# wenet-e2e/wenet

Measured on AMD Instinct MI355X. Metric: audio-seconds/sec (RTF^-1), 12L Conformer fbank80, ctc_prefix_beam_search, higher is better.
Workload: dtype f32 (feed-forward and subsampling-conv2 GEMMs: fp32 operands as three exact bf16 planes, six plane products on the bf16 matrix cores, f32 accumulate -- error <= the v_mfma_f32 kernel's, tests/test_gpu_x6.py; everything else v_mfma_f32)

## Files before the change

wenet_amd/csrc/cabi_ops.hip:

```cpp
#include "model_state.h"
#include "x6.h"

namespace wn {
namespace {

__global__ __launch_bounds__(256) void conv1_image_unpack_kernel(
    const char* __restrict__ img, int tiles, const int* __restrict__ t1_off,
    const int* __restrict__ t1_len, int F1, int C, float* __restrict__ out) {
  const int b = blockIdx.y;
  const int n = t1_len[b] * F1 * (C / 8);
  const int ne = (F1 + 1) / 2;
  for (int i = blockIdx.x * 256 + threadIdx.x; i < n; i += gridDim.x * 256) {
    const int cg = i % (C / 8), px = i / (C / 8);
    const int fr = px / F1, pos = px - fr * F1;
    const int f1 = pos < ne ? 2 * pos : 2 * (pos - ne) + 1;
    const int row = (t1_off[b] + fr) * F1;
    const char* src = img + x3_piece(cg >> 1, tiles, row + pos, cg & 1);
    const bf16x8 p0 = *reinterpret_cast<const bf16x8*>(src);
    const bf16x8 p1 = *reinterpret_cast<const bf16x8*>(src + X3_REC);
    const bf16x8 p2 = *reinterpret_cast<const bf16x8*>(src + 2 * X3_REC);
    float* o = out + ((int64_t)row + f1) * C + cg * 8;
#pragma unroll
    for (int e = 0; e < 8; ++e) o[e] = ((float)p0[e] + (float)p1[e]) + (float)p2[e];
  }
// ... 176 lines not shown
  a.B3 = w3.as<char>(); a.M = M; a.N = N; a.K = K; a.bm = bm;
  if (bm == 120) { a.bm = 128; a.nw = 8; }
  if (bm == 129) { a.bm = 128; a.nw = 4; }
  a.bias = bias; a.resid = resid; a.ldr = N; a.alpha = alpha; a.act = act; a.C = C; a.ldc = N;
  for (int r = 0; r < (reps > 0 ? reps : 1); ++r) WN_TRY(gemm_x6(a, s));
  return 0;
}

int wn_op_ffn_x6(const float* X, const float* W1, const float* b1, const float* W2,
                 const float* b2, float* x, const float* ln_w, const float* ln_b, float* y,
                 int32_t M, int32_t D, int32_t F, int32_t act, float alpha, float eps,
                 int32_t reps, void* stream) {
  WN_CHECK(X && W1 && b1 && W2 && b2 && x && ln_w && ln_b && y, "ffn_x6: null argument");
  WN_CHECK(M > 0 && (D == 256 || D == 512) && F > 0 && F % 64 == 0, "ffn_x6: shape");
  hipStream_t s = (hipStream_t)stream;
  static thread_local DevBuf x3, w13, w23, h3, part;
  if (tune().ffn_x6f != 0 && tune().x6_af32 == 0 && ffn_x6f_supported(M, D, F, act)) {
    FfnX6Args a;
    a.S = ffn_x6f_split(M, F);
    WN_TRY(w13.ensure(x6_bytes(F, D)));
    WN_TRY(w23.ensure(x6_bytes(D, F)));
    WN_TRY(part.ensure((size_t)a.S * M * D * sizeof(float)));
    WN_TRY(x6_split(W1, F, D, D, w13.as<char>(), s));
    WN_TRY(x6_split_perm(W2, D, F, F, w23.as<char>(), s));
    a.X = X; a.ldx = D; a.W13 = w13.as<char>(); a.W2p = w23.as<char>(); a.b1 = b1;
    a.P = part.as<float>(); a.M = M; a.D = D; a.F = F; a.act = act;
    if (tune().ffn_ximg == 2) {
      WN_TRY(x3.ensure(x6_bytes(M, D)));
      WN_TRY(x6_split(X, M, D, D, x3.as<char>(), s));
      a.X3 = x3.as<char>(); a.X = nullptr;
    }
    for (int r = 0; r < (reps > 0 ? reps : 1); ++r) WN_TRY(ffn_x6f(a, s));
    return ffn_reduce_ln(x, part.as<float>(), a.S, b2, alpha, ln_w, ln_b, nullptr, nullptr, y, M,
                         D, eps, 0, s);
  }
  const int S = ffn_x6_split(M, F);
  WN_TRY(x3.ensure(x6_bytes(M, D)));
  WN_TRY(w13.ensure(x6_bytes(F, D)));
  WN_TRY(w23.ensure(x6_bytes(D, F)));
  WN_TRY(h3.ensure(x6_bytes(M, F)));
  WN_TRY(part.ensure((size_t)S * M * D * sizeof(float)));
  WN_TRY(x6_split(W1, F, D, D, w13.as<char>(), s));
  WN_TRY(x6_split(W2, D, F, F, w23.as<char>(), s));
  const bool af32 = tune().x6_af32 != 0 && (int64_t)M * F * 4 < ((int64_t)1 << 31);
  static thread_local DevBuf hf;
  if (af32) WN_TRY(hf.ensure((size_t)M * F * sizeof(float)));
  for (int r = 0; r < (reps > 0 ? reps : 1); ++r) {
// ... 844 lines not shown
```

wenet_amd/csrc/conformer.hip:

```cpp
#include <algorithm>
#include "model_state.h"

namespace {
struct ProfBracket {
  wn_model* m;
  hipStream_t s;
  bool on = false;
  int record(int which) { WN_HIP(hipEventRecord(m->prof_ev[m->prof_used + which], s)); return 0; }
  int begin() {
    on = m->prof_on && (m->prof_seq++ % m->prof_stride) == 0;
    if (!on) return 0;
    if (m->prof_used + 2 > m->prof_ev.size())
      for (int i = 0; i < 64; ++i) {
        hipEvent_t e;
        WN_HIP(hipEventCreate(&e));
        m->prof_ev.push_back(e);
      }
    return record(0);
  }
  int end(double flops, const char* kernel) {
    if (!on) return 0;
    WN_TRY(record(1));
    m->prof_used += 2;
    m->prof_flops += flops;
// ... 87 lines not shown
static void* t1_image_for(wn_model* m, const Linear& w1, const Linear& w2, int act) {
  if (tune().ffn_ximg == 0) return nullptr;
  const int r = ffn_x6_route(m, w1, w2, act);
  if (r == 0 || (r == 2 && tune().x6_af32 != 0)) return nullptr;
  if (m->t1_img.ensure(x6_bytes(m->rows, m->cfg.d_model)) != 0) return nullptr;
  return m->t1_img.p;
}

static int ffn_x6_try(wn_model* m, const Linear& w1, const Linear& w2, int act, hipStream_t s) {
  const ModelData& W = *m->data;
  const int d = m->cfg.d_model, M = m->rows, F = w1.out;
  const bool ximg = m->t1_img_ok;
  m->t1_img_ok = false;
  const int route = ffn_x6_route(m, w1, w2, act);
  WN_CHECK(route != 0 || !ximg,
           "ffn_x6_try: LN(x) was left as a plane image but no six-product form takes it");
  if (route == 0) return 0;
  auto i1 = W.x6_at.find(w1.w), i2 = W.x6_at.find(w2.w);
  ProfBracket pb{m, s};
  if (route == 1) {
    FfnX6Args a;
    a.S = ffn_x6f_split(M, F);
    if (m->ffn_part.ensure((size_t)a.S * M * d * sizeof(float)) != 0) return -1;
    a.X = m->t1.as<float>(); a.ldx = d; a.W13 = i1->second; a.W2p = W.x6p_at.find(w2.w)->second;
    a.b1 = w1.b;
    if (ximg) { a.X3 = m->t1_img.p; a.X = nullptr; }
    a.P = m->ffn_part.as<float>(); a.M = M; a.D = d; a.F = F; a.act = act;
    WN_TRY(pb.begin());
    if (ffn_x6f(a, s) != 0) return -1;
    WN_TRY(pb.end(4.0 * M * (double)F * d,
                  "ffn_x6f_kernel (FFN w_1 + act + w_2, six bf16 plane products)"));
    m->prof_split = a.S;
    return a.S;
  }
  const int S = ffn_x6_split(M, F);
  if (m->ffn_part.ensure((size_t)S * M * d * sizeof(float)) != 0) return -1;
  const bool af32 = tune().x6_af32 != 0 && (int64_t)M * F * 4 < ((int64_t)1 << 31);
  X6Args g1;
  g1.B3 = i1->second; g1.M = M; g1.N = F; g1.K = d; g1.bias = w1.b; g1.act = act;
  if (af32) {
    WN_CHECK(!ximg, "ffn_x6_try: LN(x) was left as a plane image, x6_af32 wants fp32 rows");
    if (m->hbuf.ensure((size_t)M * F * sizeof(float)) != 0) return -1;
    g1.A = m->t1.as<float>(); g1.lda = d; g1.a_bytes = (int64_t)M * d * 4;
    g1.epi = 0; g1.C = m->hbuf.as<float>(); g1.ldc = F;
  } else {
    if (m->x6_h.ensure(x6_bytes(M, F)) != 0 || (!ximg && m->x6_a.ensure(x6_bytes(M, d)) != 0)) return -1;
    if (!ximg && x6_split(m->t1.as<float>(), M, d, d, m->x6_a.as<char>(), s) != 0) return -1;
// ... 424 lines not shown
```

wenet_amd/csrc/ffn_x6f.hip:

```cpp
#include <type_traits>

#include "common.h"
#include "gemm_epilogue.h"
#include "kernels.h"
#include "x6.h"

namespace wn {

namespace {

__device__ unsigned long long g_x6f_clk[4][24];

constexpr int REC = X3_REC;
constexpr int XSTAGE = 24 * REC;
constexpr int XD = 256;
constexpr int XKB = XD / 16;

typedef unsigned u32x4 __attribute__((ext_vector_type(4)));
struct Frag6 { bf16x8 p[2][3]; };

__global__ __launch_bounds__(256) void x6_split_perm_kernel(const float* __restrict__ src, int R,
                                                            int K, int ld,
                                                            char* __restrict__ dst) {
  const int tiles = (R + 31) >> 5, nkb = K >> 4;
  const int64_t idx = (int64_t)blockIdx.x * 256 + threadIdx.x;
  const int row_l = (int)(idx & 31), h = (int)((idx >> 5) & 1);
  const int64_t rest = idx >> 6;
  const int kb = (int)(rest % nkb), tile = (int)(rest / nkb);
  if (tile >= tiles) return;
  const int row = tile * 32 + row_l;
  f32x4 a = {0.f, 0.f, 0.f, 0.f}, b = a;
  if (row < R) {
    const float* s = src + (int64_t)row * ld + kb * 16 + h * 4;
    a = *reinterpret_cast<const f32x4*>(s);
    b = *reinterpret_cast<const f32x4*>(s + 8);
  }
  bf16x8 p0, p1, p2;
#pragma unroll
  for (int e = 0; e < 4; ++e) {
    const Split3 sa = split3(a[e]), sb = split3(b[e]);
    p0[e] = sa.h0; p1[e] = sa.h1; p2[e] = sa.h2;
    p0[4 + e] = sb.h0; p1[4 + e] = sb.h1; p2[4 + e] = sb.h2;
  }
  char* o = dst + ((int64_t)kb * tiles + tile) * X3_TILE + h * 512 + row_l * 16;
  *reinterpret_cast<bf16x8*>(o) = p0;
  *reinterpret_cast<bf16x8*>(o + REC) = p1;
  *reinterpret_cast<bf16x8*>(o + 2 * REC) = p2;
}

__device__ __forceinline__ void wait_vm_stages(int stages) {
  switch (stages) {
    case 0: asm volatile("s_waitcnt vmcnt(0)" ::: "memory"); break;
    case 1: asm volatile("s_waitcnt vmcnt(6)" ::: "memory"); break;
    case 2: asm volatile("s_waitcnt vmcnt(12)" ::: "memory"); break;
    case 3: asm volatile("s_waitcnt vmcnt(18)" ::: "memory"); break;
    default: asm volatile("s_waitcnt vmcnt(24)" ::: "memory"); break;
  }
}

template <int ACT, int RING, int VAR>
__global__ __launch_bounds__(256, 1) void ffn_x6f_kernel(FfnX6Args p, int tiles_m, int pairmap) {
  extern __shared__ __attribute__((aligned(16))) char smem_g[];
  typedef __attribute__((address_space(3))) void* lds_ptr;
  constexpr int HALF = (VAR & 512) ? 2 : 1;
  constexpr int STG = XSTAGE * HALF;
  constexpr int SPC = 8 / HALF;
  static_assert(RING >= 3 && RING * STG <= 6 * XSTAGE, "ring of at most 144 KB");
  float* b1s = reinterpret_cast<float*>(smem_g + RING * STG);

  const int bid = blockIdx.x, xcd = bid & 7, rr = bid >> 3;
  int slice, tm;
  if (pairmap && p.S >= 2 && p.S <= 8) {
    const int nsp = p.S >> 1, pair = xcd % nsp, tg = xcd / nsp;
    slice = 2 * pair + (rr & 1);
    tm = (rr >> 1) * (8 / nsp) + tg;
  } else if (p.S <= 8) {
    slice = xcd & (p.S - 1);
    tm = rr * (8 / p.S) + xcd / p.S;
  } else {
    const int sub = p.S >> 3;
    slice = xcd + 8 * (rr % sub);
    tm = rr / sub;
  }
  if (tm >= tiles_m) return;

  unsigned long long clk[20] = {0, 0, 0, 0, 0, 0, 0, 0, 0, 0, 0, 0, 0, 0, 0, 0, 0, 0, 0, 0};
  if constexpr ((VAR & 8192) != 0) {
    clk[9] = __builtin_readcyclecounter();
    clk[12] = __builtin_amdgcn_s_memrealtime();
  }
  const int tid = threadIdx.x, lane = tid & 63;
  const int wave = __builtin_amdgcn_readfirstlane(tid >> 6);
  __builtin_assume(wave >= 0 && wave < 4);
  const int hi = lane >> 5, li = lane & 31;
  const int NC = p.F / p.S / 64;
  const int cg0 = slice * NC;
  const int FT = p.F >> 5;
  const unsigned vlane = (unsigned)lane * 16u;

  const __amdgpu_buffer_rsrc_t r1 = __builtin_amdgcn_make_buffer_rsrc(
      const_cast<char*>(reinterpret_cast<const char*>(p.W13)), 0,
      (int)((int64_t)p.F * XD * 6), 0x00020000);
  const __amdgpu_buffer_rsrc_t r2 = __builtin_amdgcn_make_buffer_rsrc(
      const_cast<char*>(reinterpret_cast<const char*>(p.W2p)), 0,
      (int)((int64_t)p.F * XD * 6), 0x00020000);

  auto issue_sub = [&](int c, int sub, int buf) {
    char* dst = smem_g + buf * STG + (sub % HALF) * XSTAGE + wave * 6 * REC;
    const int cg = cg0 + c;
    if (sub < 4) {
      const int nt = sub >> 1;
#pragma unroll
      for (int j2 = 0; j2 < 2; ++j2) {
        const int ks = (sub & 1) * 8 + wave * 2 + j2;
        const int so = ((ks * FT + 2 * cg + nt) * 3) * REC;
#pragma unroll
        for (int pl = 0; pl < 3; ++pl)
// ... 25 lines not shown
      __builtin_amdgcn_raw_ptr_buffer_load_lds(r2, (lds_ptr)dst, 16, vlane, so + j * REC, 0, 0);
    }
  };
  auto read_group = [&](int buf, int g) {
    const char* st = smem_g + buf * STG + g * 6 * REC + lane * 16;
    Frag6 f;
#pragma unroll
    for (int t = 0; t < 2; ++t)
#pragma unroll
      for (int pl = 0; pl < 3; ++pl)
        f.p[t][pl] = *reinterpret_cast<const bf16x8*>(st + (t * 3 + pl) * REC);
    return f;
  };

  constexpr bool XT = (VAR & 16384) != 0;
  constexpr bool XI = (VAR & 32768) != 0;
  bf16x8 X[XKB][3];
  const int xrow = min(tm * 128 + wave * 32 + li, p.M - 1);
  f32x4 xa[XKB], xb[XKB];
  f32x4 xr[4][8];
  if constexpr (XI) {
    const int tiles = (p.M + 31) >> 5;
    const int tile = min(tm * 4 + wave, tiles - 1);
    const char* xi = reinterpret_cast<const char*>(p.X3) + (int64_t)tile * X3_TILE + lane * 16;
    const int64_t kstr = (int64_t)tiles * X3_TILE;
#pragma unroll
    for (int ks = 0; ks < XKB; ++ks)
#pragma unroll
      for (int pl = 0; pl < 3; ++pl)
        X[ks][pl] = *reinterpret_cast<const bf16x8*>(xi + ks * kstr + pl * REC);
  } else if constexpr (XT) {
    const int r4 = lane >> 4, c16 = lane & 15;
#pragma unroll
    for (int q = 0; q < 4; ++q)
#pragma unroll
      for (int j = 0; j < 8; ++j) {
        const int row = min(tm * 128 + wave * 32 + 4 * j + r4, p.M - 1);
        xr[q][j] = *reinterpret_cast<const f32x4*>(p.X + (int64_t)row * p.ldx + q * 64 + c16 * 4);
      }
  } else {
    const float* xr0 = p.X + (int64_t)xrow * p.ldx + hi * 8;
#pragma unroll
    for (int ks = 0; ks < XKB; ++ks) {
      xa[ks] = *reinterpret_cast<const f32x4*>(xr0 + ks * 16);
      xb[ks] = *reinterpret_cast<const f32x4*>(xr0 + ks * 16 + 4);
    }
  }
#pragma unroll
  for (int t = 0; t < ((VAR & 16384) ? RING - 1 : RING); ++t) issue(0, t, t);
  float b1v[8];
#pragma unroll
  for (int i = 0; i < 8; ++i) b1v[i] = p.b1[cg0 * 64 + min(tid + 256 * i, NC * 64 - 1)];
  if constexpr ((VAR & 8192) != 0) { __builtin_amdgcn_sched_barrier(0); clk[15] = __builtin_readcyclecounter(); __builtin_amdgcn_sched_barrier(0); }
  if constexpr (XT && !XI) {
    char* patch = smem_g + (RING - 1) * STG + wave * (32 * 272);
    const int r4 = lane >> 4, c16 = lane & 15;
#pragma unroll
    for (int q = 0; q < 4; ++q) {
#pragma unroll
      for (int j = 0; j < 8; ++j)
        *reinterpret_cast<f32x4*>(patch + (4 * j + r4) * 272 + c16 * 16) = xr[q][j];
#pragma unroll
      for (int k4 = 0; k4 < 4; ++k4) {
        xa[4 * q + k4] = *reinterpret_cast<const f32x4*>(patch + li * 272 + k4 * 64 + hi * 32);
        xb[4 * q + k4] = *reinterpret_cast<const f32x4*>(patch + li * 272 + k4 * 64 + hi * 32 + 16);
      }
      asm volatile("s_waitcnt lgkmcnt(0)" ::: "memory");
    }
  }
  if constexpr (!XI) {
#pragma unroll
    for (int ks = 0; ks < XKB; ++ks) {
#pragma unroll
      for (int e = 0; e < 4; ++e) {
        const Split3 sa = split3(xa[ks][e]), sb = split3(xb[ks][e]);
        X[ks][0][e] = sa.h0; X[ks][1][e] = sa.h1; X[ks][2][e] = sa.h2;
        X[ks][0][4 + e] = sb.h0; X[ks][1][4 + e] = sb.h1; X[ks][2][4 + e] = sb.h2;
      }
    }
  }
  if constexpr ((VAR & 8192) != 0) { __builtin_amdgcn_sched_barrier(0); clk[16] = __builtin_readcyclecounter(); __builtin_amdgcn_sched_barrier(0); }
  asm volatile("s_waitcnt vmcnt(0)" ::: "memory");
  if constexpr ((VAR & 8192) != 0) { __builtin_amdgcn_sched_barrier(0); clk[17] = __builtin_readcyclecounter(); __builtin_amdgcn_sched_barrier(0); }
#pragma unroll
  for (int ks = 0; ks < XKB; ++ks)
#pragma unroll
    for (int pl = 0; pl < 3; ++pl) asm volatile("" : "+v"(X[ks][pl]));
#pragma unroll
  for (int i = 0; i < 8; ++i)
    if (tid + 256 * i < NC * 64) b1s[tid + 256 * i] = b1v[i];
  __syncthreads();
  if constexpr ((VAR & 8192) != 0) { __builtin_amdgcn_sched_barrier(0); clk[18] = __builtin_readcyclecounter(); __builtin_amdgcn_sched_barrier(0); }

  f32x16 Y[8];
#pragma unroll
  for (int i = 0; i < 8; ++i)
#pragma unroll
    for (int r = 0; r < 16; ++r) Y[i][r] = 0.f;
  f32x16 HE[2], HO[2];
  u32x4 Hp[4][3];
  if (VAR & 4)
#pragma unroll
    for (int i = 0; i < 12; ++i) {
      Hp[i / 3][i % 3] = u32x4{0x3f803f80u, 0x3f803f80u, 0x3f803f80u, 0x3f803f80u};
      asm volatile("" : "+v"(Hp[i / 3][i % 3]));
    }

  constexpr int PW[6] = {2, 0, 1, 1, 0, 0}, PX[6] = {0, 2, 1, 0, 1, 0};
  constexpr int RT[6] = {0, 1, 0, 1, 0, 1}, RP[6] = {2, 2, 0, 0, 1, 1};

  float pv0 = 0.f, pv1 = 0.f, pt0 = 0.f, pt1 = 0.f;
  unsigned ph0 = 0, ph1 = 0;
  auto pk = [](float a, float b) {
    typedef __bf16 bf16x2 __attribute__((ext_vector_type(2)));
    const bf16x2 h = {(__bf16)a, (__bf16)b};
    return __builtin_bit_cast(unsigned, h);
  };
  auto lo = [](unsigned u) { return __builtin_bit_cast(float, u << 16); };
  auto hi16 = [](unsigned u) { return __builtin_bit_cast(float, u & 0xffff0000u); };
  auto piece_slice = [&](int nt, int i, int k, const f32x4& bq) {
    const int r = 2 * i;
    switch (k) {
      case 0: {
        float b0 = bq[r & 3];
        asm volatile("" : "+v"(b0));
        pv0 = HE[nt][r] + b0;
        break;
      }
      case 1: {
        float b1 = bq[(r + 1) & 3];
        asm volatile("" : "+v"(b1), "+v"(pv0));
        pv0 += HO[nt][r];
        pv1 = HE[nt][r + 1] + b1;
        break;
      }
      case 2:
        asm volatile("" : "+v"(pv0), "+v"(pv1));
        pv1 += HO[nt][r + 1];
        if (ACT == ACT_SILU) pt0 = pv0 * -1.4426950408889634f;
        break;
      case 3:
        if (ACT == ACT_SILU) {
          asm volatile("" : "+v"(pt0), "+v"(pv1));
          pt1 = pv1 * -1.4426950408889634f;
          pt0 = wn_exp2(pt0);
        }
        break;
      case 4:
        if (ACT == ACT_SILU) {
          asm volatile("" : "+v"(pt0), "+v"(pt1));
          pt1 = wn_exp2(pt1);
          pt0 = 1.0f + pt0;
        }
        break;
      case 5:
        if (ACT == ACT_SILU) {
          asm volatile("" : "+v"(pt0), "+v"(pt1));
          pt1 = 1.0f + pt1;
          pt0 = wn_rcp(pt0);
        }
        break;
// ... 9 lines not shown
      case 7:
        asm volatile("" : "+v"(pv0), "+v"(pv1));
        if (ACT == ACT_SILU) {
          asm volatile("" : "+v"(pt1));
          pv1 *= pt1;
        }
        if (ACT == ACT_RELU) pv1 = fmaxf(pv1, 0.0f);
        ph0 = pk(pv0, pv1);
        break;
      case 8:
        asm volatile("" : "+v"(pv0), "+v"(pv1), "+v"(ph0));
        pv0 -= lo(ph0); pv1 -= hi16(ph0);
        break;
      case 9:
        asm volatile("" : "+v"(pv0), "+v"(pv1));
        ph1 = pk(pv0, pv1);
        break;
      case 10:
        asm volatile("" : "+v"(pv0), "+v"(pv1), "+v"(ph1));
        pv0 -= lo(ph1); pv1 -= hi16(ph1);
        break;
      default: {
        asm volatile("" : "+v"(pv0), "+v"(pv1));
        const int kb = 2 * nt + (r >> 3), d = (r & 7) >> 1;
        Hp[kb][0][d] = ph0;
        Hp[kb][1][d] = ph1;
        Hp[kb][2][d] = pk(pv0, pv1);
        break;
      }
    }
  };
  auto read_frag = [&](int b, int g, int t, int pl) {
    return *reinterpret_cast<const bf16x8*>(smem_g + b * STG + (g * 6 + t * 3 + pl) * REC +
                                            lane * 16);
  };
  const f32x16 zero16 = {0.f, 0.f, 0.f, 0.f, 0.f, 0.f, 0.f, 0.f, 0.f, 0.f, 0.f, 0.f, 0.f, 0.f, 0.f,
                         0.f};

  int buf = 0;
  Frag6 fc;
#pragma unroll
  for (int q = 0; q < 6; ++q) fc.p[RT[q]][RP[q]] = read_frag(0, 0, RT[q], RP[q]);
  if constexpr ((VAR & 8192) != 0) clk[10] = __builtin_readcyclecounter();
  auto chunk = [&](auto last_tag, int c) {
    constexpr bool last = decltype(last_tag)::value;
    f32x4 bq = {0.f, 0.f, 0.f, 0.f};
#pragma unroll
    for (int sub = 0; sub < 8; ++sub) {
      if constexpr ((VAR & 8192) != 0 && !last) {
        __builtin_amdgcn_sched_barrier(0);
        clk[sub] = __builtin_readcyclecounter();
        __builtin_amdgcn_sched_barrier(0);
      }
#pragma unroll
      for (int g = 0; g < 4; ++g) {
        Frag6 fn;
        const bool do_piece = sub >= 2 && sub < 6;
        const int pnt = sub >= 4 ? 1 : 0;
        const int pi = ((sub & 1) << 2) + g;
        if (do_piece && (pi & 1) == 0)
          bq = *reinterpret_cast<const f32x4*>(b1s + c * 64 + pnt * 32 + 8 * (pi >> 1) + 4 * hi);
#pragma unroll
        for (int k = 0; k < 12; ++k) {
          const int q = k >> 1, tl = k & 1;
          if ((VAR & 1) || ((VAR & 65536) && q >= 3)) {
            asm volatile("" ::"v"(fc.p[tl][PW[q]]));
          } else if (sub < 4) {
            const int nt = sub >> 1, ks = (sub & 1) * 8 + 2 * g + tl;
            const bool first = (sub & 1) == 0 && g == 0 && q == 0;
            f32x16& H = tl == 0 ? HE[nt] : HO[nt];
            H = __builtin_amdgcn_mfma_f32_32x32x16_bf16(fc.p[tl][PW[q]], X[ks][PX[q]],
                                                       first ? zero16 : H, 0, 0, 0);
          } else {
            const bf16x8 hb = __builtin_bit_cast(bf16x8, Hp[sub - 4][PX[q]]);
            Y[2 * g + tl] = __builtin_amdgcn_mfma_f32_32x32x16_bf16(fc.p[tl][PW[q]], hb,
                                                                    Y[2 * g + tl], 0, 0, 0);
          }
          const int st = sub / HALF;
          const bool sync_sub = sub % HALF == HALF - 1;
          const int gs = (sub % HALF) * 4 + g;
          if (g == 3 && k == 5 && sync_sub) {
            __builtin_amdgcn_sched_barrier(0);
            if (!(VAR & 8)) {
              if (!(VAR & 1024)) {
                asm volatile("s_waitcnt lgkmcnt(0)" ::: "memory");
                const int tail = SPC - 2 - st < 0 ? 0 : (SPC - 2 - st > RING - 2 ? RING - 2 : SPC - 2 - st);
                if (last) wait_vm_stages(tail * HALF); else wait_vm_stages((RING - 2) * HALF);
              }
              if (!(VAR & 2048)) __builtin_amdgcn_s_barrier();
// ... 2 lines not shown
              if (st + RING < SPC) issue(c, st + RING, buf);
              else if (!last) issue(c + 1, st + RING - SPC, buf);
            }
            buf = buf + 1 == RING ? 0 : buf + 1;
            __builtin_amdgcn_sched_barrier(0);
          }
          if constexpr ((VAR & 16384) != 0 && !(VAR & 2)) {
            static_assert(!(VAR & 16384) || HALF == 2, "spread DMA: 48-record stages");
            const int ka = do_piece ? 9 : 2, kb = do_piece ? 11 : 8;
            if ((k == ka || k == kb) && gs < 6) {
              const int j12 = gs * 2 + (k == kb ? 1 : 0);
              const int tst = st + RING - 1;
              const int bufp = buf == 0 ? RING - 1 : buf - 1;
              if (tst < SPC) issue_one(c, tst * HALF + j12 / 6, bufp, j12 % 6);
              else if (!last) issue_one(c + 1, (tst - SPC) * HALF + j12 / 6, bufp, j12 % 6);
            }
          }
          if (VAR & 64) {
            fn = fc;
          } else if (g < 3 || !sync_sub) {
            if (VAR & 4096) {
              if (k == 0)
#pragma unroll
                for (int i = 0; i < 6; ++i) fn.p[RT[i]][RP[i]] = read_frag(buf, gs + 1, RT[i], RP[i]);
            } else if (tl == 1) {
              fn.p[RT[q]][RP[q]] = read_frag(buf, gs + 1, RT[q], RP[q]);
            }
          } else if (k >= 6 && (sub < 7 || !last)) {
            fn.p[RT[k - 6]][RP[k - 6]] = read_frag(buf, 0, RT[k - 6], RP[k - 6]);
          }
          if (do_piece) {
            if (VAR & 4) {
              if (k == 11) {
                const int r = 2 * pi, kb = 2 * pnt + (r >> 3), d = (r & 7) >> 1;
                Hp[kb][0][d] = __builtin_bit_cast(unsigned, HE[pnt][r]) & 0x3f803f80u;
                Hp[kb][1][d] = __builtin_bit_cast(unsigned, HO[pnt][r]) & 0x3f803f80u;
                Hp[kb][2][d] = __builtin_bit_cast(unsigned, HE[pnt][r + 1]) & 0x3f803f80u;
              }
            } else {
              piece_slice(pnt, pi, k, bq);
            }
          }
          __builtin_amdgcn_sched_barrier(0);
        }
        fc = fn;
      }
    }
    if constexpr ((VAR & 8192) != 0 && !last) clk[8] = __builtin_readcyclecounter();
  };
  for (int c = 0; c + 1 < NC; ++c) chunk(std::false_type{}, c);
  chunk(std::true_type{}, NC - 1);

  if constexpr ((VAR & 8192) != 0) clk[11] = __builtin_readcyclecounter();
  const int row = tm * 128 + wave * 32 + li;
  if constexpr (XT) {
    __syncthreads();
    char* patch = smem_g + wave * (32 * 1040);
#pragma unroll
    for (int i = 0; i < 8; ++i)
#pragma unroll
      for (int g = 0; g < 4; ++g)
        *reinterpret_cast<f32x4*>(patch + li * 1040 + (i * 32 + 8 * g + 4 * hi) * 4) =
            f32x4{Y[i][4 * g], Y[i][4 * g + 1], Y[i][4 * g + 2], Y[i][4 * g + 3]};
    float* P0 = p.P + ((int64_t)slice * p.M + tm * 128 + wave * 32) * XD + lane * 4;
    const int nrow = min(32, p.M - (tm * 128 + wave * 32));
#pragma unroll
    for (int r = 0; r < 32; ++r) {
      const f32x4 v = *reinterpret_cast<const f32x4*>(patch + r * 1040 + lane * 16);
      if (r < nrow) *reinterpret_cast<f32x4*>(P0 + (int64_t)r * XD) = v;
    }
  } else if (row < p.M) {
    float* P = p.P + ((int64_t)slice * p.M + row) * XD;
#pragma unroll
    for (int i = 0; i < 8; ++i)
#pragma unroll
      for (int g = 0; g < 4; ++g)
      {
        const f32x4 v = f32x4{Y[i][4 * g], Y[i][4 * g + 1], Y[i][4 * g + 2], Y[i][4 * g + 3]};
        float* o = P + i * 32 + 8 * g + 4 * hi;
        if (VAR & 128) asm volatile("global_store_dwordx4 %0, %1, off sc0 sc1" ::"v"(o), "v"(v) : "memory");
        else if (VAR & 256) asm volatile("global_store_dwordx4 %0, %1, off nt" ::"v"(o), "v"(v) : "memory");
        else *reinterpret_cast<f32x4*>(o) = v;
      }
  }
  if constexpr ((VAR & 8192) != 0) {
    asm volatile("s_waitcnt vmcnt(0)" ::: "memory");
    clk[13] = __builtin_amdgcn_s_memrealtime();
    const unsigned long long t_end = __builtin_readcyclecounter();
    if (blockIdx.x == gridDim.x / 2 && lane == 0) {
#pragma unroll
      for (int i = 0; i < 20; ++i) g_x6f_clk[wave][i] = clk[i];
      g_x6f_clk[wave][20] = t_end;
    }
  }
}

template <int ACT, int RING, int VAR = 0>
int launch_x6f(const FfnX6Args& a, hipStream_t s) {
  const int tiles_m = cdiv(a.M, 128);
  const int NC = a.F / a.S / 64;
  const size_t lds = (size_t)RING * XSTAGE * ((VAR & 512) ? 2 : 1) + (size_t)NC * 64 * sizeof(float);
  const int pairmap = a.S >= 2 && a.S <= 8;
  const int grid = pairmap      ? cdiv(tiles_m, 16 / a.S) * 16
                   : a.S <= 8 ? cdiv(tiles_m, 8 / a.S) * 8
                              : tiles_m * a.S;
  auto kern = ffn_x6f_kernel<ACT, RING, VAR>;
  WN_MAX_DYN_LDS(kern, 160 * 1024);
  hipLaunchKernelGGL(kern, dim3(grid), dim3(256), lds, s, a, tiles_m, pairmap);
  WN_HIP(hipGetLastError());
  return 0;
}

}


int ffn_x6f_clocks(unsigned long long* out) {
  WN_HIP(hipMemcpyFromSymbol(out, HIP_SYMBOL(g_x6f_clk), sizeof(g_x6f_clk)));
  return 0;
}

int x6_split_perm(const float* src, int R, int K, int ld, void* dst, hipStream_t s) {
  WN_CHECK(src && dst && R > 0 && K > 0 && K % 16 == 0 && ld % 4 == 0, "x6_split_perm: shape");
  const int64_t n = (int64_t)cdiv(R, 32) * (K / 16) * 64;
  hipLaunchKernelGGL(x6_split_perm_kernel, dim3((unsigned)((n + 255) / 256)), dim3(256), 0, s,
                     src, R, K, ld, reinterpret_cast<char*>(dst));
  WN_HIP(hipGetLastError());
  return 0;
}

int ffn_x6f_split(int M, int F) {
  const int tiles_m = cdiv(M, 128);
  int S = 1;
  while (S < 32 && tiles_m * (S * 2) <= 256 && F % (S * 2 * 64) == 0) S *= 2;
  return S;
}

bool ffn_x6f_supported(int M, int D, int F, int act) {
  if (D != XD || M <= 0 || F <= 0 || F % 64 != 0) return false;
  if (act != ACT_SILU && act != ACT_RELU) return false;
  const int S = ffn_x6f_split(M, F);
  if (F % (S * 64) != 0 || F / S > 2048) return false;
  if ((int64_t)cdiv(M, 32) * X3_TILE * XKB >= ((int64_t)1 << 40)) return false;
  return tune().ffn_x6f != 3 || cdiv(M, 128) * S >= 128;
}

int ffn_x6f(const FfnX6Args& a, hipStream_t s) {
  WN_CHECK((a.X3 || (a.X && a.ldx % 4 == 0)) && a.W13 && a.W2p && a.b1 && a.P && a.M > 0 && a.D == XD && a.S > 0 &&
               a.F % (a.S * 64) == 0 && a.F / a.S <= 2048 && (a.S & (a.S - 1)) == 0 && a.S <= 32,
           "ffn_x6f: bad arguments");
#define WN_X6F(RING, VAR)                                            \
  switch (a.act) {                                                   \
    case ACT_SILU: return launch_x6f<ACT_SILU, RING, VAR>(a, s);     \
    case ACT_RELU: return launch_x6f<ACT_RELU, RING, VAR>(a, s);     \
    default: break;                                                  \
  }
  if (tune().ffn_x6f_var == 25088 && a.act == ACT_SILU) {
    if (a.X3) return launch_x6f<ACT_SILU, 3, 25088 + 32768>(a, s);
    return launch_x6f<ACT_SILU, 3, 25088>(a, s);
  }
#ifdef WN_ABLATION
  if (tune().ffn_x6f_var != 0 && a.act == ACT_SILU) {
    switch (tune().ffn_x6f_var) {
      case 1: return launch_x6f<ACT_SILU, 6, 1>(a, s);
      case 2: return launch_x6f<ACT_SILU, 6, 2>(a, s);
      case 4: return launch_x6f<ACT_SILU, 6, 4>(a, s);
      case 8: return launch_x6f<ACT_SILU, 6, 8>(a, s);
      case 64: return launch_x6f<ACT_SILU, 6, 64>(a, s);
      case 10: return launch_x6f<ACT_SILU, 6, 10>(a, s);
      case 78: return launch_x6f<ACT_SILU, 6, 78>(a, s);
      case 74: return launch_x6f<ACT_SILU, 6, 74>(a, s);
      case 14: return launch_x6f<ACT_SILU, 6, 14>(a, s);
      case 76: return launch_x6f<ACT_SILU, 6, 76>(a, s);
      case 70: return launch_x6f<ACT_SILU, 6, 70>(a, s);
      case 1094: return launch_x6f<ACT_SILU, 6, 1094>(a, s);
      case 4096: return launch_x6f<ACT_SILU, 6, 4096>(a, s);
      case 4110: return launch_x6f<ACT_SILU, 6, 4110>(a, s);
      case 2118: return launch_x6f<ACT_SILU, 6, 2118>(a, s);
// ... 25 lines not shown
```

wenet_amd/csrc/kernels.h:

```cpp
#pragma once
#include "common.h"

namespace wn {

int layernorm(const float* x, int ldx, const float* w, const float* b, float* y,
              int ldy, int M, int D, float eps, hipStream_t s, bool y_bf16 = false);

int layernorm_mx(const float* x, int ldx, const float* w, const float* b, void* q,
                 unsigned* scale, int pitch, int M, int D, float eps, hipStream_t s);

int layernorm2(const float* x, const float* w1, const float* b1, const float* w2,
               const float* b2, float* y1, float* y2, int M, int D, float eps,
               hipStream_t s, bool y2_bf16 = false);

struct Conv1Args {
  const float* feats;
  const float* mean;
  const float* istd;
  const float* w;
  const float* bias;
  float* out;
  char* out3 = nullptr;
  int tiles = 0;
  const int* t1_off;
// ... 237 lines not shown
int gemm_x6_clocks(unsigned long long* out);
size_t x6_bytes(int R, int K);
int x6_split(const float* src, int R, int K, int ld, void* dst, hipStream_t s);
int gemm_x6_bm(int M, int N, int ksplit);
int gemm_x6(const X6Args& a, hipStream_t s);
enum X6ConvTile {
  X6CONV_128 = 0,
  X6CONV_256 = 1,
  X6CONV_256_REM128 = 2,
  X6CONV_256_KTAIL = 3
};
struct X6ConvForm {
  int tile = X6CONV_128;
  int full = 0;
  int slices = 0;
};
X6ConvForm gemm_x6_conv_form(const X6Args& a);
struct FfnX6Args {
  const float* X = nullptr;
  int ldx = 0;
  const void* X3 = nullptr;
  const void* W13 = nullptr;
  const void* W2p = nullptr;
  const float* b1 = nullptr;
  float* P = nullptr;
  int M = 0, D = 0, F = 0, S = 0, act = 0;
};
int ffn_x6f_clocks(unsigned long long* out);
int x6_split_perm(const float* src, int R, int K, int ld, void* dst, hipStream_t s);
int ffn_x6f_split(int M, int F);
bool ffn_x6f_supported(int M, int D, int F, int act);
int ffn_x6f(const FfnX6Args& a, hipStream_t s);


struct RowLnArgs {
  const float* A; int lda;
  const float* W;
  const float* bias;
  const float* resid; int ldr;
  float alpha;
  float* x_out; int ldx;
  const float* ln_w; const float* ln_b; float eps;
  float* y; int ldy;
  int M, N, K;
};
struct X6RArgs {
  const float* A = nullptr; int lda = 0;
  int K = 256;
  const void* W3 = nullptr;
  const float* bias = nullptr;
  int M = 0, N = 0;
  int epi = 0;
// ... 406 lines not shown
```

wenet_amd/csrc/model.hip:

```cpp
#include <algorithm>
#include "model_state.h"

namespace wn {

static thread_local std::string g_error;
void set_error(const std::string& msg) { g_error = msg; }
const char* last_error_cstr() { return g_error.c_str(); }

}

thread_local const std::map<const float*, ModelData::MxW>* t_mx = nullptr;
thread_local const std::map<const float*, const void*>* t_x6 = nullptr;
thread_local DevBuf* t_x6_a = nullptr;

namespace wn {
Tune g_tune_default;
thread_local const Tune* t_tune = nullptr;

int* tune_field(Tune& t, const std::string& key) {
#define X(name, dflt) if (key == #name) return &t.name;
  WN_TUNE_KEYS(X)
#undef X
  return nullptr;
}

int tune_check(const std::string& key, int32_t value, const char* who) {
  if (value == TUNE_INHERIT) return 0;
  if (key == "rnnt_lookahead" && (value < 1 || value > 16)) {
    set_error(std::string(who) + ": rnnt_lookahead must be in [1, 16]");
    return -1;
  }
#ifndef WN_ABLATION
  if (key == "x6_probe" && (value & ~12) != 0) {
    set_error(std::string(who) + ": x6_probe 1 / 2 (no MFMAs / no DMA) need a WN_ABLATION build");
    return -1;
  }
  if (key == "ffn_x6f_var" && value != 0 && value != 25088) {
    set_error(std::string(who) + ": ffn_x6f_var variants other than the clock-stamp form "
              "(25088) need a WN_ABLATION build");
    return -1;
  }
  if (key == "attn_x6_var" && value != 0) {
    set_error(std::string(who) + ": attn_x6_var needs a WN_ABLATION build");
    return -1;
  }
  if (key == "ffn_x6f_ring" && value != 3) {
    set_error(std::string(who) + ": ffn_x6f_ring needs a WN_ABLATION build");
    return -1;
  }
#endif
  return 0;
}

void tune_resolve(const Tune& ovr, Tune* eff) {
#define X(name, dflt) eff->name = ovr.name != TUNE_INHERIT ? ovr.name : g_tune_default.name;
  WN_TUNE_KEYS(X)
// ... 89 lines not shown
  for (const Decoder* D : {&W.left, &W.right})
    if (D->out.w) vocab.push_back(&D->out);
  for (const Linear* l : vocab) ws.push_back(l);
  size_t bytes = 0;
  for (const Linear* l : ws)
    if (l->w && l->in % 16 == 0) bytes += x6_bytes(l->out, l->in);
  if (bytes > 0) {
    WN_TRY(W.weights_x6.ensure(bytes));
    char* p = W.weights_x6.as<char>();
    for (const Linear* l : ws) {
      if (!l->w || l->in % 16 != 0 || W.x6_at.count(l->w)) continue;
      WN_TRY(x6_split(l->w, l->out, l->in, l->in, p, nullptr));
      W.x6_at[l->w] = p;
      p += x6_bytes(l->out, l->in);
    }
  }
  if (cfg.d_model == 256) {
    std::vector<const Linear*> w2s;
    for (const auto& L : enc_layers) { w2s.push_back(&L.ffm2); w2s.push_back(&L.ff2); }
    size_t pbytes = 0;
    for (const Linear* l : w2s)
      if (l->w && l->in % 64 == 0 && l->out == 256) pbytes += x6_bytes(l->out, l->in);
    if (pbytes > 0) {
      WN_TRY(W.weights_x6p.ensure(pbytes));
      char* q = W.weights_x6p.as<char>();
      for (const Linear* l : w2s) {
        if (!l->w || l->in % 64 != 0 || l->out != 256 || W.x6p_at.count(l->w)) continue;
        WN_TRY(x6_split_perm(l->w, l->out, l->in, l->in, q, nullptr));
        W.x6p_at[l->w] = q;
        q += x6_bytes(l->out, l->in);
      }
    }
  }
  if (cfg.d_model == 256 && cfg.n_heads == 4) {
    size_t n_q = 0;
    for (const auto& L : enc_layers)
      if (L.qkv.w && L.qkv.b && L.qkv.out == 768 && L.qkv.in == 256 && L.pos_tab) ++n_q;
    if (n_q > 0) {
      const size_t img = x6_bytes(768, 256), per = img + 768 * sizeof(float);
      DevBuf stage;
      WN_TRY(stage.ensure((size_t)768 * 256 * sizeof(float)));
      WN_TRY(W.weights_x6q.ensure(n_q * per));
      char* q = W.weights_x6q.as<char>();
      for (const auto& L : enc_layers) {
        if (!(L.qkv.w && L.qkv.b && L.qkv.out == 768 && L.qkv.in == 256 && L.pos_tab) ||
            W.x6q_at.count(L.qkv.w))
          continue;
        float* qb = reinterpret_cast<float*>(q + img);
        for (int h = 0; h < 4; ++h)
          for (int part = 0; part < 3; ++part) {
            const size_t nr = (size_t)h * 192 + part * 64, orow = (size_t)part * 256 + h * 64;
            WN_HIP(hipMemcpyAsync(stage.as<float>() + nr * 256, L.qkv.w + orow * 256,
// ... 525 lines not shown
```

wenet_amd/csrc/model_state.h:

```cpp
#pragma once
#include <math.h>
#include <stdio.h>
#include <stdlib.h>
#include <string.h>

#include <atomic>
#include <chrono>
#include <map>
#include <memory>
#include <mutex>
#include <string>
#include <vector>

#include "../../include/wenet_amd.h"
#include "kernels.h"

namespace wn {

const char* last_error_cstr();


struct DevBuf {
  void* p = nullptr;
  size_t cap = 0;
// ... 158 lines not shown
};

struct Decoder {
  const float* embed = nullptr;
  const float* pe = nullptr;
  float xscale = 1.0f;
  int max_pos = 0;
  Norm after;
  Linear out;
  std::vector<DecLayer> layers;
};
}

using namespace wn;


struct ModelData {
  DevBuf weights;
  int64_t n_weight_elems = 0;
  DevBuf weights_x6;
  std::map<const float*, const void*> x6_at;
  DevBuf weights_x6p;
  std::map<const float*, const void*> x6p_at;
  DevBuf weights_x6q;
  std::map<const float*, std::pair<const void*, const float*>> x6q_at;
  DevBuf bias4_buf;
  std::map<const float*, const float*> bias4;
  std::map<std::string, const float*> w;
  const float* conv1_w = nullptr; const float* conv1_b = nullptr;
  Linear conv2, sub_out;
  const float* cmvn_mean = nullptr; const float* cmvn_istd = nullptr;
  const float* pe = nullptr;
  Norm after_norm;
  Linear ctc;
  std::vector<EncLayer> layers;
  std::vector<TfLayer> tf_layers;
  Linear tconv1, tconv2;
  bool fbank_ok = true;
  Decoder left, right;
  DevBuf pos_tabs;
  struct LstmLayer { const float* w_ih; const float* w_hh; const float* b_ih; const float* b_hh; };
  const float* pred_embed = nullptr;
  std::vector<LstmLayer> pred_rnn;
  Linear pred_proj, j_enc, j_pred, j_out;
  const float* pred_pos = nullptr;
  const float* pred_conv_w = nullptr; const float* pred_conv_b = nullptr;
// ... 284 lines not shown
```

wenet_amd/csrc/tune.h:

```cpp
#pragma once
#include <stdint.h>

#include <string>

namespace wn {

#define WN_TUNE_KEYS(X)                                                                         \
                          \
  X(gemm_tile_bf16, 0)                                                                          \
                            \
  X(bf16_store, 1)                                                                              \
                      \
  X(lp_probe, 0)                                                                                \
                       \
  X(attn_split, 0)                                                                              \
                     \
  X(attn_bf16, 1)                                                                               \
                 \
  X(attn_bf16_nw, 0)                                                                            \
                                                                            \
  X(attn_bf16_defer, 80)                                                                        \
                                                              \
  X(attn_bf16_dma, 1)                                                                           \
                        \
// ... 4 lines not shown
  X(ffn_fused, 1)                                                                               \
                                                                   \
  X(gemm_x6, 1)                                                                                 \
                                         \
  X(x6_linear, 1)                                                                               \
                      \
  X(x6_af32, 0)                                                                                 \
            \
  X(x6_conv_af32, 0)                                                                            \
     \
  X(enc_gate_pos, 0)                                                                            \
                                                            \
  X(x6_conv_bm, 128)                                                                            \
                    \
  X(x6_probe, 0)                                                                                \
                     \
  X(ffn_x6f, 1)                                                                                 \
            \
  X(ffn_ximg, 1)                                                                                \
                             \
  X(ffn_x6f_ring, 3)                                                                            \
                  \
  X(ffn_x6f_var, 0)                                                                             \
                                                                        \
  X(x6r, 1)                                                                                     \
                  \
  X(x6r_chain, 1)                                                                               \
          \
  X(x6r_dwc, 1)                                                                                 \
        \
  X(x6r_pro, 1)                                                                                 \
            \
  X(x6r512_rows, 0)                                                                             \
                 \
  X(gemm_rowln, 1)                                                                              \
          \
  X(dwconv_tiled, 1)                                                                            \
                               \
  X(attn_x6, 1)                                                                                 \
                   \
  X(attn_xcd, 1)                                                                                \
        \
  X(attn_x6_galign, 2)                                                                          \
                             \
  X(attn_x6_order, 1)                                                                           \
    \
// ... 39 lines not shown
```

Measured before the change: 71560.

## Add 16x16x32 bf16 MFMA form to fused FFN six-product kernel

Adds an alternative instruction form for the fused FFN kernel that uses 16x16x32 bf16 MFMAs instead of 32x32x16. The weight and activation plane images, LDS fragment reads and epilogue writes are re-laid out to match, and a second permuted copy of W2 is precomputed at model load. The new form is on by default through a tune key. The aim is better MFMA throughput or scheduling on MI355X. In exchange it doubles the W2 plane image memory and adds register arrays and layout complexity.

```diff
diff --git a/wenet_amd/csrc/cabi_ops.hip b/wenet_amd/csrc/cabi_ops.hip
--- a/wenet_amd/csrc/cabi_ops.hip
+++ b/wenet_amd/csrc/cabi_ops.hip
@@ -222,7 +222,8 @@
     WN_TRY(w23.ensure(x6_bytes(D, F)));
     WN_TRY(part.ensure((size_t)a.S * M * D * sizeof(float)));
     WN_TRY(x6_split(W1, F, D, D, w13.as<char>(), s));
-    WN_TRY(x6_split_perm(W2, D, F, F, w23.as<char>(), s));
+    a.mfma = ffn_x6f_form();
+    WN_TRY(x6_split_perm(W2, D, F, F, w23.as<char>(), s, a.mfma));
     a.X = X; a.ldx = D; a.W13 = w13.as<char>(); a.W2p = w23.as<char>(); a.b1 = b1;
     a.P = part.as<float>(); a.M = M; a.D = D; a.F = F; a.act = act;
     if (tune().ffn_ximg == 2) {
diff --git a/wenet_amd/csrc/conformer.hip b/wenet_amd/csrc/conformer.hip
--- a/wenet_amd/csrc/conformer.hip
+++ b/wenet_amd/csrc/conformer.hip
@@ -133,7 +133,8 @@
     FfnX6Args a;
     a.S = ffn_x6f_split(M, F);
     if (m->ffn_part.ensure((size_t)a.S * M * d * sizeof(float)) != 0) return -1;
-    a.X = m->t1.as<float>(); a.ldx = d; a.W13 = i1->second; a.W2p = W.x6p_at.find(w2.w)->second;
+    a.X = m->t1.as<float>(); a.ldx = d; a.W13 = i1->second; a.mfma = ffn_x6f_form();
+    a.W2p = (a.mfma == 16 ? W.x6p16_at : W.x6p_at).find(w2.w)->second;
     a.b1 = w1.b;
     if (ximg) { a.X3 = m->t1_img.p; a.X = nullptr; }
     a.P = m->ffn_part.as<float>(); a.M = M; a.D = d; a.F = F; a.act = act;
diff --git a/wenet_amd/csrc/ffn_x6f.hip b/wenet_amd/csrc/ffn_x6f.hip
--- a/wenet_amd/csrc/ffn_x6f.hip
+++ b/wenet_amd/csrc/ffn_x6f.hip
@@ -21,7 +21,7 @@
 
 __global__ __launch_bounds__(256) void x6_split_perm_kernel(const float* __restrict__ src, int R,
                                                             int K, int ld,
-                                                            char* __restrict__ dst) {
+                                                            char* __restrict__ dst, int form) {
   const int tiles = (R + 31) >> 5, nkb = K >> 4;
   const int64_t idx = (int64_t)blockIdx.x * 256 + threadIdx.x;
   const int row_l = (int)(idx & 31), h = (int)((idx >> 5) & 1);
@@ -31,9 +31,10 @@
   const int row = tile * 32 + row_l;
   f32x4 a = {0.f, 0.f, 0.f, 0.f}, b = a;
   if (row < R) {
-    const float* s = src + (int64_t)row * ld + kb * 16 + h * 4;
+    const float* s = src + (int64_t)row * ld +
+                     (form == 16 ? (kb >> 1) * 32 + (kb & 1) * 8 + h * 4 : kb * 16 + h * 4);
     a = *reinterpret_cast<const f32x4*>(s);
-    b = *reinterpret_cast<const f32x4*>(s + 8);
+    b = *reinterpret_cast<const f32x4*>(s + (form == 16 ? 16 : 8));
   }
   bf16x8 p0, p1, p2;
 #pragma unroll
@@ -58,8 +59,10 @@
   }
 }
 
-template <int ACT, int RING, int VAR>
+template <int ACT, int RING, int VAR, int MF>
 __global__ __launch_bounds__(256, 1) void ffn_x6f_kernel(FfnX6Args p, int tiles_m, int pairmap) {
+  static_assert(MF == 32 || (MF == 16 && (VAR & 512) && (VAR & 16384) && !(VAR & 4096)),
+                "16x16x32 form: 48-record stages, rows through the patch");
   extern __shared__ __attribute__((aligned(16))) char smem_g[];
   typedef __attribute__((address_space(3))) void* lds_ptr;
   constexpr int HALF = (VAR & 512) ? 2 : 1;
@@ -93,6 +96,7 @@
   const int wave = __builtin_amdgcn_readfirstlane(tid >> 6);
   __builtin_assume(wave >= 0 && wave < 4);
   const int hi = lane >> 5, li = lane & 31;
+  const int q4 = lane >> 4, r16 = lane & 15;
   const int NC = p.F / p.S / 64;
   const int cg0 = slice * NC;
   const int FT = p.F >> 5;
@@ -164,13 +168,24 @@
   if constexpr (XI) {
     const int tiles = (p.M + 31) >> 5;
     const int tile = min(tm * 4 + wave, tiles - 1);
-    const char* xi = reinterpret_cast<const char*>(p.X3) + (int64_t)tile * X3_TILE + lane * 16;
     const int64_t kstr = (int64_t)tiles * X3_TILE;
-#pragma unroll
-    for (int ks = 0; ks < XKB; ++ks)
-#pragma unroll
-      for (int pl = 0; pl < 3; ++pl)
-        X[ks][pl] = *reinterpret_cast<const bf16x8*>(xi + ks * kstr + pl * REC);
+    if constexpr (MF == 16) {
+      const char* xi = reinterpret_cast<const char*>(p.X3) + (int64_t)tile * X3_TILE +
+                       (q4 >> 1) * kstr + (q4 & 1) * 512 + r16 * 16;
+#pragma unroll
+      for (int ks = 0; ks < XKB; ++ks)
+#pragma unroll
+        for (int pl = 0; pl < 3; ++pl)
+          X[ks][pl] = *reinterpret_cast<const bf16x8*>(xi + (ks >> 1) * 2 * kstr + pl * REC +
+                                                       (ks & 1) * 256);
+    } else {
+      const char* xi = reinterpret_cast<const char*>(p.X3) + (int64_t)tile * X3_TILE + lane * 16;
+#pragma unroll
+      for (int ks = 0; ks < XKB; ++ks)
+#pragma unroll
+        for (int pl = 0; pl < 3; ++pl)
+          X[ks][pl] = *reinterpret_cast<const bf16x8*>(xi + ks * kstr + pl * REC);
+    }
   } else if constexpr (XT) {
     const int r4 = lane >> 4, c16 = lane & 15;
 #pragma unroll
@@ -204,8 +219,10 @@
         *reinterpret_cast<f32x4*>(patch + (4 * j + r4) * 272 + c16 * 16) = xr[q][j];
 #pragma unroll
       for (int k4 = 0; k4 < 4; ++k4) {
-        xa[4 * q + k4] = *reinterpret_cast<const f32x4*>(patch + li * 272 + k4 * 64 + hi * 32);
-        xb[4 * q + k4] = *reinterpret_cast<const f32x4*>(patch + li * 272 + k4 * 64 + hi * 32 + 16);
+        const char* pr = MF == 16 ? patch + ((k4 & 1) * 16 + r16) * 272 + (k4 >> 1) * 128 + q4 * 32
+                                  : patch + li * 272 + k4 * 64 + hi * 32;
+        xa[4 * q + k4] = *reinterpret_cast<const f32x4*>(pr);
+        xb[4 * q + k4] = *reinterpret_cast<const f32x4*>(pr + 16);
       }
       asm volatile("s_waitcnt lgkmcnt(0)" ::: "memory");
     }
@@ -234,11 +251,16 @@
   __syncthreads();
   if constexpr ((VAR & 8192) != 0) { __builtin_amdgcn_sched_barrier(0); clk[18] = __builtin_readcyclecounter(); __builtin_amdgcn_sched_barrier(0); }
 
-  f32x16 Y[8];
-#pragma unroll
-  for (int i = 0; i < 8; ++i)
+  f32x16 Y[MF == 16 ? 1 : 8];
+#pragma unroll
+  for (int i = 0; i < (MF == 16 ? 1 : 8); ++i)
 #pragma unroll
     for (int r = 0; r < 16; ++r) Y[i][r] = 0.f;
+  f32x4 Y4[MF == 16 ? 8 : 1][2][2], H4[2][2][2];
+#pragma unroll
+  for (int i = 0; i < (MF == 16 ? 8 : 1); ++i)
+#pragma unroll
+    for (int r = 0; r < 4; ++r) Y4[i][r >> 1][r & 1] = f32x4{0.f, 0.f, 0.f, 0.f};
   f32x16 HE[2], HO[2];
   u32x4 Hp[4][3];
   if (VAR & 4)
@@ -262,23 +284,29 @@
   auto hi16 = [](unsigned u) { return __builtin_bit_cast(float, u & 0xffff0000u); };
   auto piece_slice = [&](int nt, int i, int k, const f32x4& bq) {
     const int r = 2 * i;
+    const f32x4& h4 = H4[nt][i >> 2][(i >> 1) & 1];
     switch (k) {
       case 0: {
         float b0 = bq[r & 3];
         asm volatile("" : "+v"(b0));
-        pv0 = HE[nt][r] + b0;
+        if constexpr (MF == 16) pv0 = h4[r & 3] + b0;
+        else pv0 = HE[nt][r] + b0;
         break;
       }
       case 1: {
         float b1 = bq[(r + 1) & 3];
         asm volatile("" : "+v"(b1), "+v"(pv0));
-        pv0 += HO[nt][r];
-        pv1 = HE[nt][r + 1] + b1;
+        if constexpr (MF == 16) {
+          pv1 = h4[(r & 3) + 1] + b1;
+        } else {
+          pv0 += HO[nt][r];
+          pv1 = HE[nt][r + 1] + b1;
+        }
         break;
       }
       case 2:
         asm volatile("" : "+v"(pv0), "+v"(pv1));
-        pv1 += HO[nt][r + 1];
+        if constexpr (MF != 16) pv1 += HO[nt][r + 1];
         if (ACT == ACT_SILU) pt0 = pv0 * -1.4426950408889634f;
         break;
       case 3:
@@ -334,7 +362,8 @@
         break;
       default: {
         asm volatile("" : "+v"(pv0), "+v"(pv1));
-        const int kb = 2 * nt + (r >> 3), d = (r & 7) >> 1;
+        const int kb = MF == 16 ? 2 * nt + ((i >> 1) & 1) : 2 * nt + (r >> 3);
+        const int d = MF == 16 ? 2 * (i >> 2) + (i & 1) : (r & 7) >> 1;
         Hp[kb][0][d] = ph0;
         Hp[kb][1][d] = ph1;
         Hp[kb][2][d] = pk(pv0, pv1);
@@ -342,9 +371,20 @@
       }
     }
   };
-  auto read_frag = [&](int b, int g, int t, int pl) {
-    return *reinterpret_cast<const bf16x8*>(smem_g + b * STG + (g * 6 + t * 3 + pl) * REC +
-                                            lane * 16);
+  const int off16a = (q4 >> 1) * 3 * REC + (q4 & 1) * 512 + r16 * 16;
+  const int off16b = (q4 >> 1) * XSTAGE + (q4 & 1) * 512 + r16 * 16;
+  auto read_frag = [&](int b, bool wb, int g, int t, int pl) {
+    if constexpr (MF == 16)
+      return *reinterpret_cast<const bf16x8*>(smem_g + b * STG + (wb ? (g * 3 + pl) * REC + off16b
+                                                                     : (g * 6 + pl) * REC + off16a) +
+                                              t * 256);
+    else
+      return *reinterpret_cast<const bf16x8*>(smem_g + b * STG + (g * 6 + t * 3 + pl) * REC +
+                                              lane * 16);
+  };
+  const f32x4 zero4 = {0.f, 0.f, 0.f, 0.f};
+  auto mfma16 = [](const bf16x8& a, const bf16x8& b, const f32x4& c) {
+    return __builtin_amdgcn_mfma_f32_16x16x32_bf16(a, b, c, 0, 0, 0);
   };
   const f32x16 zero16 = {0.f, 0.f, 0.f, 0.f, 0.f, 0.f, 0.f, 0.f, 0.f, 0.f, 0.f, 0.f, 0.f, 0.f, 0.f,
                          0.f};
@@ -352,7 +392,7 @@
   int buf = 0;
   Frag6 fc;
 #pragma unroll
-  for (int q = 0; q < 6; ++q) fc.p[RT[q]][RP[q]] = read_frag(0, 0, RT[q], RP[q]);
+  for (int q = 0; q < 6; ++q) fc.p[RT[q]][RP[q]] = read_frag(0, false, 0, RT[q], RP[q]);
   if constexpr ((VAR & 8192) != 0) clk[10] = __builtin_readcyclecounter();
   auto chunk = [&](auto last_tag, int c) {
     constexpr bool last = decltype(last_tag)::value;
@@ -371,12 +411,29 @@
         const int pnt = sub >= 4 ? 1 : 0;
         const int pi = ((sub & 1) << 2) + g;
         if (do_piece && (pi & 1) == 0)
-          bq = *reinterpret_cast<const f32x4*>(b1s + c * 64 + pnt * 32 + 8 * (pi >> 1) + 4 * hi);
+          bq = *reinterpret_cast<const f32x4*>(
+              b1s + c * 64 + pnt * 32 + (MF == 16 ? 16 * (pi >> 2) + 4 * q4 : 8 * (pi >> 1) + 4 * hi));
 #pragma unroll
         for (int k = 0; k < 12; ++k) {
           const int q = k >> 1, tl = k & 1;
           if ((VAR & 1) || ((VAR & 65536) && q >= 3)) {
             asm volatile("" ::"v"(fc.p[tl][PW[q]]));
+          } else if (MF == 16) {
+            if (sub < 4) {
+              const int nt = sub >> 1, ks = (sub & 1) * 8 + 2 * g;
+              const bool first = (sub & 1) == 0 && g == 0 && q == 0;
+#pragma unroll
+              for (int u = 0; u < 2; ++u)
+                H4[nt][tl][u] = mfma16(fc.p[tl][PW[q]], X[ks + u][PX[q]],
+                                       first ? zero4 : H4[nt][tl][u]);
+            } else {
+              const int v = (sub - 4) >> 1, dt = (sub & 1) * 4 + g;
+#pragma unroll
+              for (int u = 0; u < 2; ++u)
+                Y4[dt][tl][u] = mfma16(fc.p[tl][PW[q]],
+                                       __builtin_bit_cast(bf16x8, Hp[2 * v + u][PX[q]]),
+                                       Y4[dt][tl][u]);
+            }
           } else if (sub < 4) {
             const int nt = sub >> 1, ks = (sub & 1) * 8 + 2 * g + tl;
             const bool first = (sub & 1) == 0 && g == 0 && q == 0;
@@ -425,12 +482,12 @@
             if (VAR & 4096) {
               if (k == 0)
 #pragma unroll
-                for (int i = 0; i < 6; ++i) fn.p[RT[i]][RP[i]] = read_frag(buf, gs + 1, RT[i], RP[i]);
+                for (int i = 0; i < 6; ++i) fn.p[RT[i]][RP[i]] = read_frag(buf, sub >= 4, gs + 1, RT[i], RP[i]);
             } else if (tl == 1) {
-              fn.p[RT[q]][RP[q]] = read_frag(buf, gs + 1, RT[q], RP[q]);
+              fn.p[RT[q]][RP[q]] = read_frag(buf, sub >= 4, gs + 1, RT[q], RP[q]);
             }
           } else if (k >= 6 && (sub < 7 || !last)) {
-            fn.p[RT[k - 6]][RP[k - 6]] = read_frag(buf, 0, RT[k - 6], RP[k - 6]);
+            fn.p[RT[k - 6]][RP[k - 6]] = read_frag(buf, sub >= 3 && sub < 7, 0, RT[k - 6], RP[k - 6]);
           }
           if (do_piece) {
             if (VAR & 4) {
@@ -459,12 +516,23 @@
   if constexpr (XT) {
     __syncthreads();
     char* patch = smem_g + wave * (32 * 1040);
-#pragma unroll
-    for (int i = 0; i < 8; ++i)
-#pragma unroll
-      for (int g = 0; g < 4; ++g)
-        *reinterpret_cast<f32x4*>(patch + li * 1040 + (i * 32 + 8 * g + 4 * hi) * 4) =
-            f32x4{Y[i][4 * g], Y[i][4 * g + 1], Y[i][4 * g + 2], Y[i][4 * g + 3]};
+    if constexpr (MF == 16) {
+#pragma unroll
+      for (int i = 0; i < 8; ++i)
+#pragma unroll
+        for (int t = 0; t < 2; ++t)
+#pragma unroll
+          for (int u = 0; u < 2; ++u)
+            *reinterpret_cast<f32x4*>(patch + (16 * u + r16) * 1040 +
+                                      (i * 32 + 16 * t + 4 * q4) * 4) = Y4[i][t][u];
+    } else {
+#pragma unroll
+      for (int i = 0; i < 8; ++i)
+#pragma unroll
+        for (int g = 0; g < 4; ++g)
+          *reinterpret_cast<f32x4*>(patch + li * 1040 + (i * 32 + 8 * g + 4 * hi) * 4) =
+              f32x4{Y[i][4 * g], Y[i][4 * g + 1], Y[i][4 * g + 2], Y[i][4 * g + 3]};
+    }
     float* P0 = p.P + ((int64_t)slice * p.M + tm * 128 + wave * 32) * XD + lane * 4;
     const int nrow = min(32, p.M - (tm * 128 + wave * 32));
 #pragma unroll
@@ -498,7 +566,7 @@
   }
 }
 
-template <int ACT, int RING, int VAR = 0>
+template <int ACT, int RING, int VAR = 0, int MF = 32>
 int launch_x6f(const FfnX6Args& a, hipStream_t s) {
   const int tiles_m = cdiv(a.M, 128);
   const int NC = a.F / a.S / 64;
@@ -507,7 +575,7 @@
   const int grid = pairmap      ? cdiv(tiles_m, 16 / a.S) * 16
                    : a.S <= 8 ? cdiv(tiles_m, 8 / a.S) * 8
                               : tiles_m * a.S;
-  auto kern = ffn_x6f_kernel<ACT, RING, VAR>;
+  auto kern = ffn_x6f_kernel<ACT, RING, VAR, MF>;
   WN_MAX_DYN_LDS(kern, 160 * 1024);
   hipLaunchKernelGGL(kern, dim3(grid), dim3(256), lds, s, a, tiles_m, pairmap);
   WN_HIP(hipGetLastError());
@@ -522,11 +590,12 @@
   return 0;
 }
 
-int x6_split_perm(const float* src, int R, int K, int ld, void* dst, hipStream_t s) {
+int x6_split_perm(const float* src, int R, int K, int ld, void* dst, hipStream_t s, int form) {
   WN_CHECK(src && dst && R > 0 && K > 0 && K % 16 == 0 && ld % 4 == 0, "x6_split_perm: shape");
+  WN_CHECK(form == 32 || (form == 16 && K % 32 == 0), "x6_split_perm: form");
   const int64_t n = (int64_t)cdiv(R, 32) * (K / 16) * 64;
   hipLaunchKernelGGL(x6_split_perm_kernel, dim3((unsigned)((n + 255) / 256)), dim3(256), 0, s,
-                     src, R, K, ld, reinterpret_cast<char*>(dst));
+                     src, R, K, ld, reinterpret_cast<char*>(dst), form);
   WN_HIP(hipGetLastError());
   return 0;
 }
@@ -536,6 +605,14 @@
   int S = 1;
   while (S < 32 && tiles_m * (S * 2) <= 256 && F % (S * 2 * 64) == 0) S *= 2;
   return S;
+}
+
+int ffn_x6f_form() {
+#ifdef WN_ABLATION
+  if ((tune().ffn_x6f_var != 0 && tune().ffn_x6f_var != 25088) || tune().ffn_x6f_ring != 3)
+    return 32;
+#endif
+  return tune().ffn_x6f_mfma == 16 ? 16 : 32;
 }
 
 bool ffn_x6f_supported(int M, int D, int F, int act) {
@@ -551,11 +628,22 @@
   WN_CHECK((a.X3 || (a.X && a.ldx % 4 == 0)) && a.W13 && a.W2p && a.b1 && a.P && a.M > 0 && a.D == XD && a.S > 0 &&
                a.F % (a.S * 64) == 0 && a.F / a.S <= 2048 && (a.S & (a.S - 1)) == 0 && a.S <= 32,
            "ffn_x6f: bad arguments");
-#define WN_X6F(RING, VAR)                                            \
-  switch (a.act) {                                                   \
-    case ACT_SILU: return launch_x6f<ACT_SILU, RING, VAR>(a, s);     \
-    case ACT_RELU: return launch_x6f<ACT_RELU, RING, VAR>(a, s);     \
-    default: break;                                                  \
+  WN_CHECK(a.mfma == 32 || a.mfma == 16, "ffn_x6f: W2p is the image of form 32 or 16");
+#define WN_X6F(RING, VAR, ...)                                                    \
+  switch (a.act) {                                                                \
+    case ACT_SILU: return launch_x6f<ACT_SILU, RING, VAR, ##__VA_ARGS__>(a, s);   \
+    case ACT_RELU: return launch_x6f<ACT_RELU, RING, VAR, ##__VA_ARGS__>(a, s);   \
+    default: break;                                                               \
+  }
+  if (a.mfma == 16) {
+    if (tune().ffn_x6f_var == 25088 && a.act == ACT_SILU) {
+      if (a.X3) return launch_x6f<ACT_SILU, 3, 25088 + 32768, 16>(a, s);
+      return launch_x6f<ACT_SILU, 3, 25088, 16>(a, s);
+    }
+    if (a.X3) { WN_X6F(3, 16896 + 32768, 16) }
+    WN_X6F(3, 16896, 16)
+    set_error("ffn_x6f: unsupported activation");
+    return -1;
   }
   if (tune().ffn_x6f_var == 25088 && a.act == ACT_SILU) {
     if (a.X3) return launch_x6f<ACT_SILU, 3, 25088 + 32768>(a, s);
diff --git a/wenet_amd/csrc/kernels.h b/wenet_amd/csrc/kernels.h
--- a/wenet_amd/csrc/kernels.h
+++ b/wenet_amd/csrc/kernels.h
@@ -283,12 +283,14 @@
   const void* X3 = nullptr;
   const void* W13 = nullptr;
   const void* W2p = nullptr;
+  int mfma = 32;
   const float* b1 = nullptr;
   float* P = nullptr;
   int M = 0, D = 0, F = 0, S = 0, act = 0;
 };
 int ffn_x6f_clocks(unsigned long long* out);
-int x6_split_perm(const float* src, int R, int K, int ld, void* dst, hipStream_t s);
+int x6_split_perm(const float* src, int R, int K, int ld, void* dst, hipStream_t s, int form = 32);
+int ffn_x6f_form();
 int ffn_x6f_split(int M, int F);
 bool ffn_x6f_supported(int M, int D, int F, int act);
 int ffn_x6f(const FfnX6Args& a, hipStream_t s);
diff --git a/wenet_amd/csrc/model.hip b/wenet_amd/csrc/model.hip
--- a/wenet_amd/csrc/model.hip
+++ b/wenet_amd/csrc/model.hip
@@ -30,8 +30,12 @@
     set_error(std::string(who) + ": rnnt_lookahead must be in [1, 16]");
     return -1;
   }
+  if (key == "ffn_x6f_mfma" && value != 32 && value != 16) {
+    set_error(std::string(who) + ": ffn_x6f_mfma is 32 (32x32x16 MFMAs) or 16 (16x16x32)");
+    return -1;
+  }
 #ifndef WN_ABLATION
-  if (key == "x6_probe" && (value & ~12) != 0) {
+  if (key == "x6_probe"&& (value & ~12) != 0) {
     set_error(std::string(who) + ": x6_probe 1 / 2 (no MFMAs / no DMA) need a WN_ABLATION build");
     return -1;
   }
@@ -167,12 +171,15 @@
     for (const Linear* l : w2s)
       if (l->w && l->in % 64 == 0 && l->out == 256) pbytes += x6_bytes(l->out, l->in);
     if (pbytes > 0) {
-      WN_TRY(W.weights_x6p.ensure(pbytes));
+      WN_TRY(W.weights_x6p.ensure(2 * pbytes));
       char* q = W.weights_x6p.as<char>();
       for (const Linear* l : w2s) {
         if (!l->w || l->in % 64 != 0 || l->out != 256 || W.x6p_at.count(l->w)) continue;
         WN_TRY(x6_split_perm(l->w, l->out, l->in, l->in, q, nullptr));
         W.x6p_at[l->w] = q;
+        q += x6_bytes(l->out, l->in);
+        WN_TRY(x6_split_perm(l->w, l->out, l->in, l->in, q, nullptr, 16));
+        W.x6p16_at[l->w] = q;
         q += x6_bytes(l->out, l->in);
       }
     }
diff --git a/wenet_amd/csrc/model_state.h b/wenet_amd/csrc/model_state.h
--- a/wenet_amd/csrc/model_state.h
+++ b/wenet_amd/csrc/model_state.h
@@ -204,6 +204,7 @@
   std::map<const float*, const void*> x6_at;
   DevBuf weights_x6p;
   std::map<const float*, const void*> x6p_at;
+  std::map<const float*, const void*> x6p16_at;
   DevBuf weights_x6q;
   std::map<const float*, std::pair<const void*, const float*>> x6q_at;
   DevBuf bias4_buf;
diff --git a/wenet_amd/csrc/tune.h b/wenet_amd/csrc/tune.h
--- a/wenet_amd/csrc/tune.h
+++ b/wenet_amd/csrc/tune.h
@@ -50,6 +50,8 @@
   X(ffn_x6f_ring, 3)                                                                            \
                   \
   X(ffn_x6f_var, 0)                                                                             \
+                                                  \
+  X(ffn_x6f_mfma, 16)                                                                           \
                                                                         \
   X(x6r, 1)                                                                                     \
                   \
```

Measured after the change: 72230, median of 6. About the same (+0.9%).
